# dariopagliaricci/Metal-PathTracer-arm64

Measured on AMD Instinct MI355X. Metric: Msamples/sec (whole node) at 1920×1080, depth 8; PFM RMSE vs Embree ref, higher is better.
Workload: dtype f32; 1 GPU; BASELINE configs[1]: Cornell box + one 70,688-triangle OBJ mesh, 1920x1080, depth 8, 256 spp, seed 1337; partition=8-row bands round-robin over 1 rank(s), RCCL gather of the HDR buffer

## Files before the change

### metal-pathtracer-arm64_amd/csrc/host/bvh_builder.cpp

```cpp
#include "bvh_builder.h"

#include <algorithm>
#include <atomic>
#include <cmath>
#include <chrono>
#include <cstdio>
#include <cstdlib>
#include <cstring>
#include <limits>
#include <memory>
#include <numeric>
#include <thread>
#include <stdexcept>

#if defined(__SSE2__)
#include <emmintrin.h>
#endif

#include "../kernels/bvh_layout.h"
#include "knobs.h"
#include "parallel.h"

namespace ptr {
namespace {
// ... 730 lines not shown
    for (int a = 0; a < 3; ++a) {
        const double extent = static_cast<double>(scene.hi[a]) - scene.lo[a];
        cell[a] = extent > 0.0 ? extent / 65531.0 : 1.0;
        out.gridCell[a] = static_cast<float>(cell[a]);
        out.gridOrigin[a] = static_cast<float>(scene.lo[a] - 2.0 * cell[a]);
    }
    out.qnodes.assign(static_cast<size_t>(out.nodeCount) * 8, 0u);
    auto quant = [&](float v, int axis, bool up) -> uint32_t {
        const double g = (static_cast<double>(v) - out.gridOrigin[axis]) / static_cast<double>(out.gridCell[axis]);
        const double q = up ? std::ceil(g) + 1.0 : std::floor(g) - 1.0;
        return static_cast<uint32_t>(std::min(std::max(q, 0.0), 65535.0));
    };
    auto quantiseRange = [&](uint32_t begin, uint32_t end) {
        for (uint32_t i = begin; i < end; ++i) {
            const float* n = out.nodes.data() + static_cast<size_t>(i) * 16;
            uint32_t* q = out.qnodes.data() + static_cast<size_t>(i) * 8;
            for (int c = 0; c < 2; ++c) {
                const float* lo = n + c * 8;
                const float* hi = n + c * 8 + 4;
                uint32_t ref;
                std::memcpy(&ref, n + (c == 0 ? 3 : 7), 4);
                uint32_t* w = q + c * 4;
                if (ref == ptrk::kRefEmpty) {
                    w[0] = w[1] = w[2] = 0u;
                } else {
                    w[0] = quant(lo[0], 0, false) | (quant(lo[1], 1, false) << 16);
                    w[1] = quant(lo[2], 2, false) | (quant(hi[0], 0, true) << 16);
                    w[2] = quant(hi[1], 1, true) | (quant(hi[2], 2, true) << 16);
                }
                w[3] = ref;
            }
        }
    };
    {
        const uint32_t workers = out.nodeCount >= (1u << 16) ? std::min(threads, 32u) : 1u;
        const uint32_t chunk = (out.nodeCount + workers - 1) / workers;
        runOnThreads(workers, [&](uint32_t t) {
            const uint32_t lo = std::min(out.nodeCount, chunk * t), hi = std::min(out.nodeCount, chunk * (t + 1));
            if (lo < hi) quantiseRange(lo, hi);
        });
    }
    double extentSum = 0.0;
    for (uint32_t i = 0; i < n; ++i) {
        const BuildPrim& p = prims[i];
        if (!oversize[i]) extentSum += std::max(std::max(p.hi[0] - p.lo[0], p.hi[1] - p.lo[1]), p.hi[2] - p.lo[2]);
    }
    out.meanPrimExtent = static_cast<float>(extentSum / std::max(inTree, 1u));
    lap("quantise");
}

namespace {

void emptyWidePlace(uint32_t* rec) {
    rec[0] = 0xFFFFFFFFu;
    rec[1] = 0x0000FFFFu;
    rec[2] = 0x00000000u;
    rec[3] = ptrk::kRefEmpty;
}

struct WideChoice {
    const uint32_t* rec[4];
    uint32_t count = 0;
};
inline bool internalRef(uint32_t ref, uint32_t nodeCount) { return ref != ptrk::kRefEmpty && !(ref & ptrk::kRefLeafBit) && ref < nodeCount; }
inline double quantArea(const uint32_t* rec, const float* cell) {
    const double x = (static_cast<double>(rec[1] >> 16) - (rec[0] & 0xFFFFu)) * cell[0];
    const double y = (static_cast<double>(rec[2] & 0xFFFFu) - (rec[0] >> 16)) * cell[1];
    const double z = (static_cast<double>(rec[2] >> 16) - (rec[1] & 0xFFFFu)) * cell[2];
    return x * y + y * z + z * x;
}
WideChoice chooseWideChildren(const uint32_t* q, uint32_t nodeCount, const float* cell, uint32_t n, bool byArea) {
    WideChoice c;
    auto childrenOf = [&](uint32_t node, const uint32_t** dst) {
        uint32_t got = 0;
        for (uint32_t side = 0; side < 2u; ++side) {
            const uint32_t* rec = q + static_cast<size_t>(node) * 8u + side * 4u;
            if (rec[3] != ptrk::kRefEmpty) dst[got++] = rec;
        }
        return got;
    };
    c.count = childrenOf(n, c.rec);
    if (!byArea) {
        WideChoice g;
        for (uint32_t k = 0; k < c.count; ++k) {
            if (internalRef(c.rec[k][3], nodeCount)) g.count += childrenOf(c.rec[k][3], g.rec + g.count);
            else g.rec[g.count++] = c.rec[k];
        }
        return g;
    }
    while (c.count < 4u) {
        int best = -1;
        double bestArea = -1.0;
        for (uint32_t k = 0; k < c.count; ++k) {
            if (!internalRef(c.rec[k][3], nodeCount)) continue;
            const double a = quantArea(c.rec[k], cell);
            if (a > bestArea) {
                bestArea = a;
                best = static_cast<int>(k);
            }
        }
        if (best < 0) break;
        const uint32_t* two[2];
        const uint32_t got = childrenOf(c.rec[best][3], two);
        if (got == 0u) break;
        c.rec[best] = two[0];
        if (got > 1u) c.rec[c.count++] = two[1];
    }
    return c;
}

}

uint32_t BuildWideNodes(const FlatBvh& bvh, WideCollapse how, std::unique_ptr<uint32_t[]>& wide, uint32_t* depthOut) {
    const uint32_t* q = bvh.qnodes.data();
    const uint32_t nodeCount = bvh.nodeCount;
    constexpr uint32_t kNotWide = 0xFFFFFFFFu;
    if (depthOut) *depthOut = 0u;
    if (nodeCount == 0 || bvh.qnodes.size() < static_cast<size_t>(nodeCount) * 8u) return 0;
    const bool byArea = how == WideCollapse::ByArea;
    std::unique_ptr<uint32_t[]> wideIndex(new uint32_t[nodeCount]);
    std::vector<uint8_t> depth(nodeCount, 0);
    depth[0] = 1u;
    uint32_t maxDepth = 1u;
    for (uint32_t n = 0; n < nodeCount; ++n) {
        if (depth[n] == 0u) continue;
        const WideChoice c = chooseWideChildren(q, nodeCount, bvh.gridCell, n, byArea);
        for (uint32_t k = 0; k < c.count; ++k) {
            const uint32_t ref = c.rec[k][3];
            if (internalRef(ref, nodeCount)) {
                depth[ref] = static_cast<uint8_t>(std::min<uint32_t>(depth[n] + 1u, 255u));
                maxDepth = std::max<uint32_t>(maxDepth, depth[ref]);
            }
        }
    }
    if (depthOut) *depthOut = maxDepth;
    uint32_t wideCount = 0;
    for (uint32_t n = 0; n < nodeCount; ++n) wideIndex[n] = depth[n] ? wideCount++ : kNotWide;
    wide.reset(new uint32_t[static_cast<size_t>(wideCount) * 16u]);
    const uint32_t workers = nodeCount >= (1u << 16) ? std::min(32u, std::max(1u, std::thread::hardware_concurrency())) : 1u;
    auto collapse = [&](uint32_t begin, uint32_t end) {
        for (uint32_t n = begin; n < end; ++n) {
            if (wideIndex[n] == kNotWide) continue;
            uint32_t* w = wide.get() + static_cast<size_t>(wideIndex[n]) * 16u;
            const WideChoice c = chooseWideChildren(q, nodeCount, bvh.gridCell, n, byArea);
            for (uint32_t k = 0; k < c.count; ++k) {
                uint32_t* dst = w + 4u * k;
                std::memcpy(dst, c.rec[k], 16);
                if (internalRef(dst[3], nodeCount)) dst[3] = wideIndex[dst[3]];
            }
            for (uint32_t k = c.count; k < 4u; ++k) emptyWidePlace(w + 4u * k);
        }
    };
    const uint32_t chunk = (nodeCount + workers - 1u) / workers;
    runOnThreads(workers, [&](uint32_t k) {
        const uint32_t b = std::min(nodeCount, chunk * k), e = std::min(nodeCount, chunk * (k + 1u));
        if (b < e) collapse(b, e);
    });
    return wideCount;
}

}
```

### metal-pathtracer-arm64_amd/csrc/host/cabi_host.cpp

```cpp
#include <algorithm>
#include <cmath>
#include <cstdio>
#include <cstring>
#include <exception>
#include <filesystem>
#include <memory>
#include <string>
#include <vector>

#include "env_importance_sampler.h"
#include "headless.h"
#include "image_decoders.h"
#include "image_writer.h"
#include "ptr_abi.h"
#include "ptr_debug.h"
#include "scene_geometry.h"
#include "bvh_layout.h"
#include "tangent_space.h"
#include "scene_manager.h"

struct PtrHostScene {
    ptr::SceneResources resources;
    ptr::RenderSettings settings;
    PtrSceneDesc desc{};
// ... 269 lines not shown
            for (int a = 0; a < 3; ++a) inv[a] = 1.0 / (d[a] != 0.0 ? d[a] : 1e-300);
            auto testLeaf = [&](uint32_t ref) {
                const uint32_t first = ref & ptrk::kRefOffsetMask, count = ((ref >> ptrk::kRefCountShift) & 0xFu) % ptrk::kMaxLeafPrims + 1u;
                for (uint32_t k = 0; k < count; ++k) {
                    ++prims;
                    if (ref & ptrk::kRefSphereBit) {
                        const float* sp = &geo.sphereData[static_cast<size_t>(first + k) * 4];
                        double c[3], dd = 0, b = 0, cc = 0;
                        for (int a = 0; a < 3; ++a) { c[a] = sp[a] - o[a]; dd += d[a] * d[a]; b += c[a] * d[a]; cc += c[a] * c[a]; }
                        const double disc = b * b - dd * (cc - static_cast<double>(sp[3]) * sp[3]);
                        if (disc < 0) continue;
                        const double sq = std::sqrt(disc);
                        double t = (b - sq) / dd;
                        if (t < tmin) t = (b + sq) / dd;
                        if (t >= tmin && t <= tfar) { tfar = t; hit = true; }
                    } else {
                        const float* t3 = &geo.triData[static_cast<size_t>(first + k) * 12];
                        const double v0[3] = {t3[0], t3[1], t3[2]}, e1[3] = {t3[4], t3[5], t3[6]}, e2[3] = {t3[8], t3[9], t3[10]};
                        const double ng[3] = {e2[1] * e1[2] - e2[2] * e1[1], e2[2] * e1[0] - e2[0] * e1[2], e2[0] * e1[1] - e2[1] * e1[0]};
                        const double c[3] = {v0[0] - o[0], v0[1] - o[1], v0[2] - o[2]};
                        const double rr[3] = {c[1] * d[2] - c[2] * d[1], c[2] * d[0] - c[0] * d[2], c[0] * d[1] - c[1] * d[0]};
                        const double den = ng[0] * d[0] + ng[1] * d[1] + ng[2] * d[2];
                        if (den == 0.0) continue;
                        const double sgn = den < 0 ? -1.0 : 1.0, ad = std::fabs(den);
                        const double U = (rr[0] * e2[0] + rr[1] * e2[1] + rr[2] * e2[2]) * sgn, V = (rr[0] * e1[0] + rr[1] * e1[1] + rr[2] * e1[2]) * sgn;
                        if (U < 0 || V < 0 || U + V > ad) continue;
                        const double T = (ng[0] * c[0] + ng[1] * c[1] + ng[2] * c[2]) * sgn;
                        if (!(ad * tmin < T && T <= ad * tfar)) continue;
                        tfar = T / ad;
                        hit = true;
                    }
                }
            };
            stack.clear();
            if (bvh.oversizeRef != ptrk::kRefEmpty) testLeaf(bvh.oversizeRef);
            if (bvh.rootRef != ptrk::kRefEmpty) stack.push_back(bvh.rootRef);
            while (!stack.empty()) {
                const uint32_t ref = stack.back();
                stack.pop_back();
                if (ref & ptrk::kRefLeafBit) {
                    testLeaf(ref);
                    continue;
                }
                ++steps;
                if (levels >= 5u) {
                    const uint32_t* w = wideNodes.get() + static_cast<size_t>(ref) * 16u;
                    double entry[4];
                    uint32_t order[4], on = 0, refs[4];
                    for (uint32_t k = 0; k < 4u; ++k) {
                        const uint32_t* rec = w + 4u * k;
                        refs[k] = rec[3];
                        if (rec[3] == ptrk::kRefEmpty) continue;
                        ++boxes;
                        const double lo[3] = {bvh.gridOrigin[0] + double(rec[0] & 0xFFFFu) * bvh.gridCell[0], bvh.gridOrigin[1] + double(rec[0] >> 16) * bvh.gridCell[1],
                                              bvh.gridOrigin[2] + double(rec[1] & 0xFFFFu) * bvh.gridCell[2]};
                        const double hi[3] = {bvh.gridOrigin[0] + double(rec[1] >> 16) * bvh.gridCell[0], bvh.gridOrigin[1] + double(rec[2] & 0xFFFFu) * bvh.gridCell[1],
                                              bvh.gridOrigin[2] + double(rec[2] >> 16) * bvh.gridCell[2]};
                        double t0 = tmin, t1 = tfar;
                        for (int a = 0; a < 3; ++a) {
                            const double ta = (lo[a] - o[a]) * inv[a], tb = (hi[a] - o[a]) * inv[a];
                            t0 = std::max(t0, std::min(ta, tb));
                            t1 = std::min(t1, std::max(ta, tb));
                        }
                        if (t0 <= t1) {
                            entry[k] = t0;
                            order[on++] = k;
                        }
                    }
                    std::sort(order, order + on, [&](uint32_t a, uint32_t b) { return entry[a] > entry[b]; });
                    for (uint32_t k = 0; k < on; ++k) stack.push_back(refs[order[k]]);
                    continue;
                }
                Child kids[8];
                uint32_t kn = 0;
                auto children = [&](uint32_t node, Child* dst) {
                    const float* nd = &bvh.nodes[static_cast<size_t>(node) * 16];
                    uint32_t c = 0;
                    for (int sl = 0; sl < 2; ++sl) {
                        const uint32_t cref = bits(nd[sl == 0 ? 3 : 7]);
                        if (cref != ptrk::kRefEmpty) dst[c++] = Child{nd + sl * 8, nd + sl * 8 + 4, cref};
                    }
                    return c;
                };
                kn = children(ref, kids);
                if (levels == 4u) {
                    auto area = [](const Child& c) {
                        const double x = double(c.hi[0]) - c.lo[0], y = double(c.hi[1]) - c.lo[1], z = double(c.hi[2]) - c.lo[2];
                        return x * y + y * z + z * x;
                    };
                    while (kn < 4u) {
                        int best = -1;
                        for (uint32_t k = 0; k < kn; ++k) {
                            if (!(kids[k].ref & ptrk::kRefLeafBit) && (best < 0 || area(kids[k]) > area(kids[best]))) best = static_cast<int>(k);
                        }
                        if (best < 0) break;
                        Child two[2];
                        const uint32_t got = children(kids[best].ref, two);
                        kids[best] = two[0];
                        if (got > 1u) kids[kn++] = two[1];
                    }
                }
                for (uint32_t l = 1; l < levels && levels != 4u; ++l) {
                    Child next[8];
                    uint32_t nn = 0;
                    for (uint32_t k = 0; k < kn; ++k) {
                        if (kids[k].ref & ptrk::kRefLeafBit) next[nn++] = kids[k];
                        else nn += children(kids[k].ref, next + nn);
                    }
                    std::memcpy(kids, next, sizeof(Child) * nn);
                    kn = nn;
// ... 31 lines not shown
```

### metal-pathtracer-arm64_amd/csrc/host/geometry_cache.cpp

```cpp
#include "geometry_cache.h"

#include <cstdio>
#include <cstring>
#include <vector>

namespace ptr {

namespace {

constexpr uint64_t kMagic = 0x3330454743525450ull;

struct Header {
    uint64_t magic, fingerprint;
    uint64_t nodes, qnodes, triOrder, sphereOrder, triData, triNormals, sphereData, sphereInfo, triUv, triTangent, rectTriLeaf, wideWords;
    float gridOrigin[3], gridCell[3], meanPrimExtent;
    uint32_t rootRef, oversizeRef, nodeCount, leafCount, maxDepth, maxLeafSize, triCount, sphereCount, useQuantized, wideCount, wideDepth, pad0;
    double sahCost, gatherSeconds, buildSeconds, flattenSeconds;
};

void fnv(uint64_t& h, const void* data, size_t bytes) {
    const unsigned char* p = static_cast<const unsigned char*>(data);
    for (size_t i = 0; i < bytes; ++i) {
        h ^= p[i];
        h *= 0x100000001b3ull;
    }
}

void fnvSampled(uint64_t& h, const void* data, size_t bytes) {
    const unsigned char* p = static_cast<const unsigned char*>(data);
    if (!p) return;
    const size_t piece = 4096;
    if (bytes <= 3 * piece) {
        fnv(h, p, bytes);
        return;
    }
    fnv(h, p, piece);
    fnv(h, p + (bytes / 2 / 16) * 16, piece);
    fnv(h, p + bytes - piece, piece);
}

template <typename T>
bool put(std::FILE* f, const T* data, uint64_t count) {
    return count == 0 || std::fwrite(data, sizeof(T), count, f) == count;
}

template <typename T>
bool get(std::FILE* f, std::vector<T>& v, uint64_t count) {
    v.resize(count);
    return count == 0 || std::fread(v.data(), sizeof(T), count, f) == count;
}

}

uint64_t SceneFingerprint(const PtrSceneDesc& desc) {
    uint64_t h = 0xcbf29ce484222325ull;
    fnv(h, &desc.meshCount, sizeof(desc.meshCount));
    for (uint32_t m = 0; m < desc.meshCount; ++m) {
        const PtrMeshDesc& mesh = desc.meshes[m];
        fnv(h, &mesh.vertexCount, sizeof(mesh.vertexCount));
        fnv(h, &mesh.indexCount, sizeof(mesh.indexCount));
        fnv(h, mesh.localToWorld, sizeof(mesh.localToWorld));
        fnv(h, &mesh.materialIndex, sizeof(mesh.materialIndex));
        fnvSampled(h, mesh.positions, static_cast<size_t>(mesh.vertexCount) * 12u);
// ... 129 lines not shown
```

### metal-pathtracer-arm64_amd/csrc/host/scene_geometry.cpp

```cpp
#include "scene_geometry.h"

#include <algorithm>
#include <atomic>
#include <chrono>
#include <cmath>
#include <cstdio>
#include <cstdlib>
#include <cstring>
#include <functional>
#include <thread>

#include "../kernels/bvh_layout.h"
#include "knobs.h"
#include "parallel.h"
#include "vecmath.h"

namespace ptr {
namespace {

struct M4 {
    float m[4][4];
};

M4 loadM4(const float* p) {
// ... 379 lines not shown
            } else {
                continue;
            }
            const float* lo = n + c * 8;
            const float* hi = n + c * 8 + 4;
            bool inside = true;
            for (int a = 0; a < 3; ++a) inside = inside && b.lo[a] >= lo[a] && b.hi[a] <= hi[a];
            if (!inside) out.boxViolations += 1;
            grow(subtree[ii], b.lo);
            grow(subtree[ii], b.hi);
            if (q) {
                const uint32_t* w = q + c * 4;
                const uint32_t qlo[3] = {w[0] & 0xFFFFu, w[0] >> 16, w[1] & 0xFFFFu};
                const uint32_t qhi[3] = {w[1] >> 16, w[2] & 0xFFFFu, w[2] >> 16};
                bool ok = (w[3] == ref);
                for (int a = 0; a < 3; ++a) {
                    const double dlo = static_cast<double>(bvh.gridOrigin[a]) + static_cast<double>(qlo[a]) * bvh.gridCell[a];
                    const double dhi = static_cast<double>(bvh.gridOrigin[a]) + static_cast<double>(qhi[a]) * bvh.gridCell[a];
                    ok = ok && dlo <= lo[a] && dhi >= hi[a];
                }
                if (!ok) out.quantViolations += 1;
            }
        }
    }
    if (bvh.oversizeRef != ptrk::kRefEmpty) {
        Box b{{inf, inf, inf}, {-inf, -inf, -inf}};
        if (!(bvh.oversizeRef & ptrk::kRefLeafBit) || (bvh.oversizeRef & ptrk::kRefSphereBit)) out.badRefs += 1;
        leafBounds(bvh.oversizeRef, b);
        out.oversize = ((bvh.oversizeRef >> ptrk::kRefCountShift) & 0xFu) + 1u;
    }
    for (uint8_t s : triSeen) out.unreferenced += (s == 0);
    for (uint8_t s : sphSeen) out.unreferenced += (s == 0);

    for (int pass = 0; pass < 2 && nodeCount > 0 && !bvh.qnodes.empty(); ++pass) {
        std::unique_ptr<uint32_t[]> wide;
        uint32_t wideDepth = 0;
        const uint32_t wideCount = BuildWideNodes(bvh, pass == 0 ? WideCollapse::ByArea : WideCollapse::ByLevel, wide, &wideDepth);
        if (pass == 0) {
            out.wideNodes = wideCount;
            out.wideDepth = wideDepth;
        }
        std::vector<uint8_t> triWide(g.triCount, 0), sphWide(g.sphereCount, 0), visited(wideCount, 0);
        std::vector<uint32_t> stack{0u};
        while (!stack.empty()) {
            const uint32_t n = stack.back();
            stack.pop_back();
            if (n >= wideCount || visited[n]++) {
                out.wideProblems += 1;
                continue;
            }
            for (uint32_t c = 0; c < 4u; ++c) {
                const uint32_t* rec = &wide[static_cast<size_t>(n) * 16u + c * 4u];
                const uint32_t ref = rec[3];
                const bool inverted = (rec[0] & 0xFFFFu) > (rec[1] >> 16) && (rec[0] >> 16) > (rec[2] & 0xFFFFu) && (rec[1] & 0xFFFFu) > (rec[2] >> 16);
                const bool ordered = (rec[0] & 0xFFFFu) <= (rec[1] >> 16) && (rec[0] >> 16) <= (rec[2] & 0xFFFFu) && (rec[1] & 0xFFFFu) <= (rec[2] >> 16);
                if ((ref == ptrk::kRefEmpty) ? !inverted : !ordered) out.wideProblems += 1;
                if (ref == ptrk::kRefEmpty) continue;
                if (!(ref & ptrk::kRefLeafBit)) {
                    stack.push_back(ref);
                    continue;
                }
                const uint32_t first = ref & ptrk::kRefOffsetMask, count = ((ref >> ptrk::kRefCountShift) & 0xFu) + 1u;
                std::vector<uint8_t>& seen = (ref & ptrk::kRefSphereBit) ? sphWide : triWide;
                for (uint32_t i = first; i < first + count; ++i) {
                    if (i >= seen.size() || seen[i]++) out.wideProblems += 1;
                }
            }
        }
        for (uint32_t n = 0; n < wideCount; ++n) out.wideProblems += (visited[n] == 0);
        const uint32_t outside = bvh.oversizeRef != ptrk::kRefEmpty ? ((bvh.oversizeRef >> ptrk::kRefCountShift) & 0xFu) + 1u : 0u;
        uint64_t missed = 0;
        for (uint8_t s : triWide) missed += (s == 0);
        for (uint8_t s : sphWide) missed += (s == 0);
        if (missed != outside) out.wideProblems += 1 + (missed > outside ? missed - outside : outside - missed);
    }
}

}
```

### metal-pathtracer-arm64_amd/csrc/kernels/traverse.h

```cpp
#pragma once

#include "device_types.h"
#include "vec.h"

namespace ptrk {

struct TraceCounters {
    uint32_t nodes;
    uint32_t prims;
    uint32_t waveNodeSteps = 0, wavePrimSteps = 0, leaves = 0;
};

typedef __attribute__((address_space(3))) uint32_t LdsWord;

struct LaneStack {
    LdsWord* lds;
    uint32_t* spill;
    uint32_t spillStride;
    uint32_t limit;
    uint32_t sp;
    __device__ __forceinline__ uint32_t* spillSlot(uint32_t level) const {
        const uint32_t column = blockIdx.x * kTraceBlock + threadIdx.x;
        return spill + static_cast<size_t>(level - kLdsStackLevels) * spillStride + column;
    }
    __device__ __forceinline__ void push(uint32_t v) {
        if (sp < kLdsStackLevels) {
            lds[sp * kTraceBlock] = v;
        } else if (sp < limit) {
            *spillSlot(sp) = v;
        } else {
            return;
        }
        ++sp;
    }
    __device__ __forceinline__ uint32_t pop() {
        --sp;
        return (sp < kLdsStackLevels) ? lds[sp * kTraceBlock] : *spillSlot(sp);
    }
};

typedef uint32_t u32x4 __attribute__((ext_vector_type(4)));

struct SceneMem {
    __amdgpu_buffer_rsrc_t nodes;
    __amdgpu_buffer_rsrc_t tris;
    __amdgpu_buffer_rsrc_t wide;
};

__device__ __forceinline__ SceneMem sceneMem(const SceneView& sc) {
    SceneMem m;
    const void* nodes = sc.useQuantized ? static_cast<const void*>(sc.qnodes) : static_cast<const void*>(sc.nodes);
    m.nodes = __builtin_amdgcn_make_buffer_rsrc(const_cast<void*>(nodes), 0, sc.nodeBytes, 0x00020000);
    m.tris = __builtin_amdgcn_make_buffer_rsrc(const_cast<float4*>(sc.tris), 0, sc.triBytes, 0x00020000);
    m.wide = __builtin_amdgcn_make_buffer_rsrc(const_cast<uint4*>(sc.wnodes), 0, sc.wideBytes, 0x00020000);
    return m;
}

__device__ __forceinline__ uint4 load16u(__amdgpu_buffer_rsrc_t r, uint32_t byteOffset) {
    const u32x4 v = __builtin_amdgcn_raw_buffer_load_b128(r, byteOffset, 0, 0);
    return make_uint4(v.x, v.y, v.z, v.w);
}
__device__ __forceinline__ float4 load16f(__amdgpu_buffer_rsrc_t r, uint32_t byteOffset) {
    const u32x4 v = __builtin_amdgcn_raw_buffer_load_b128(r, byteOffset, 0, 0);
    return make_float4(__uint_as_float(v.x), __uint_as_float(v.y), __uint_as_float(v.z), __uint_as_float(v.w));
}

struct TraceHit {
    float t;
    uint32_t prim;
};

typedef float v2f __attribute__((ext_vector_type(2)));

__device__ __forceinline__ bool slabTest(f3 lo, f3 hi, f3 oi, f3 inv, float tnear, float tfar, float& entry) {
    const v2f tx = __builtin_elementwise_fma((v2f){lo.x, hi.x}, (v2f){inv.x, inv.x}, (v2f){-oi.x, -oi.x});
    const v2f ty = __builtin_elementwise_fma((v2f){lo.y, hi.y}, (v2f){inv.y, inv.y}, (v2f){-oi.y, -oi.y});
    const v2f tz = __builtin_elementwise_fma((v2f){lo.z, hi.z}, (v2f){inv.z, inv.z}, (v2f){-oi.z, -oi.z});
    const float ax = tx.x, bx = tx.y, ay = ty.x, by = ty.y, az = tz.x, bz = tz.y;
    const float t0 = fmaxf(fmaxf(fminf(ax, bx), fminf(ay, by)), fmaxf(fminf(az, bz), tnear));
    const float t1 = fminf(fminf(fmaxf(ax, bx), fmaxf(ay, by)), fminf(fmaxf(az, bz), tfar));
    entry = t0;
    return t0 <= t1 * 1.0000004f;
}

__device__ __forceinline__ bool slabTestOrdered(f3 nearQ, f3 farQ, f3 oi, f3 inv, float tnear, float tfar, float& entry) {
    const v2f tx = __builtin_elementwise_fma((v2f){nearQ.x, farQ.x}, (v2f){inv.x, inv.x}, (v2f){-oi.x, -oi.x});
    const v2f ty = __builtin_elementwise_fma((v2f){nearQ.y, farQ.y}, (v2f){inv.y, inv.y}, (v2f){-oi.y, -oi.y});
    const v2f tz = __builtin_elementwise_fma((v2f){nearQ.z, farQ.z}, (v2f){inv.z, inv.z}, (v2f){-oi.z, -oi.z});
    const float t0 = fmaxf(fmaxf(tx.x, ty.x), fmaxf(tz.x, tnear));
    const float t1 = fminf(fminf(tx.y, ty.y), fminf(tz.y, tfar));
    entry = t0;
    return t0 <= t1 * 1.0000004f;
}

__device__ __forceinline__ bool triangleTest(f3 v0, f3 e1, f3 e2, f3 org, f3 dir, float tnear, float tfar,
                                             float& t, float& u, float& v) {
    const f3 Ng = cross(e2, e1);
    const f3 C = v0 - org;
    const f3 R = cross(C, dir);
    const float den = dot(Ng, dir);
    const float absDen = fabsf(den);
    const float sgn = signbit(den) ? -1.0f : 1.0f;
    const float U = dot(R, e2) * sgn;
    const float V = dot(R, e1) * sgn;
    if (!(den != 0.0f && U >= 0.0f && V >= 0.0f && (U + V) <= absDen)) return false;
    const float T = dot(Ng, C) * sgn;
    if (!(absDen * tnear < T && T <= absDen * tfar)) return false;
    const float rcpAbsDen = 1.0f / absDen;
    t = T * rcpAbsDen;
    u = U * rcpAbsDen;
    v = V * rcpAbsDen;
    return true;
}

__device__ __forceinline__ void triangleUv(f3 v0, f3 e1, f3 e2, f3 org, f3 dir, float& u, float& v) {
    const f3 Ng = cross(e2, e1);
    const f3 C = v0 - org;
    const f3 R = cross(C, dir);
    const float den = dot(Ng, dir);
    const float absDen = fabsf(den);
    const float sgn = signbit(den) ? -1.0f : 1.0f;
    const float U = dot(R, e2) * sgn;
    const float V = dot(R, e1) * sgn;
    const float rcpAbsDen = 1.0f / absDen;
    u = U * rcpAbsDen;
    v = V * rcpAbsDen;
}

__device__ __forceinline__ bool sphereTest(float4 s, f3 org, f3 dir, float tnear, float tfar, float& t) {
    const float rd2 = 1.0f / dot(dir, dir);
    const f3 c0 = mk3(s) - org;
    const float projC0 = dot(c0, dir) * rd2;
    const f3 perp = c0 - projC0 * dir;
    const float l2 = dot(perp, perp);
    const float r2 = s.w * s.w;
    if (!(l2 <= r2)) return false;
    const float td = sqrtf((r2 - l2) * rd2);
    const float tFront = projC0 - td;
    const float tBack = projC0 + td;
    const bool validFront = (tnear <= tFront) && (tFront <= tfar);
    const bool validBack = (tnear <= tBack) && (tBack <= tfar);
    if (!validFront && !validBack) return false;
    t = validFront ? tFront : tBack;
    return true;
}

struct Trav {
    f3 org, dir, inv;
    f3 oi;
    uint32_t selX, selY, selZ;
    float tnear;
    TraceHit hit;
    uint32_t cur;
    uint32_t leafPos;
    bool anyHit;
};

template <int NODES = -1>
__device__ __forceinline__ bool travBegin(const SceneView& sc, Trav& t, f3 org, f3 dir, float tnear, float tfar, bool anyHit,
                                          LaneStack& stack) {
    t.org = org;
    t.dir = dir;
    constexpr float kInvMax = 1.0e28f;
    t.inv = mk3(fminf(fmaxf(__builtin_amdgcn_rcpf(dir.x), -kInvMax), kInvMax), fminf(fmaxf(__builtin_amdgcn_rcpf(dir.y), -kInvMax), kInvMax),
                fminf(fmaxf(__builtin_amdgcn_rcpf(dir.z), -kInvMax), kInvMax));
    if (NODES >= 1 || (NODES < 0 && sc.useQuantized)) {
        const f3 cell = mk3(sc.gridCell[0], sc.gridCell[1], sc.gridCell[2]);
        const f3 invCell = mk3(sc.gridInvCell[0], sc.gridInvCell[1], sc.gridInvCell[2]);
        const f3 orgQ = (org - mk3(sc.gridOrigin[0], sc.gridOrigin[1], sc.gridOrigin[2])) * invCell;
        t.inv = t.inv * cell;
        t.oi = orgQ * t.inv;
    } else {
        t.oi = org * t.inv;
    }
    t.selX = t.inv.x < 0.0f ? 0x01000706u : 0x07060100u;
    t.selY = t.inv.y < 0.0f ? 0x03020504u : 0x05040302u;
    t.selZ = t.inv.z < 0.0f ? 0x01000706u : 0x07060100u;
    t.tnear = tnear;
    t.hit.t = tfar;
    t.hit.prim = kHitMiss;
    t.anyHit = anyHit;
    t.cur = sc.rootRef;
    t.leafPos = 0u;
    stack.sp = 0;
    if (sc.oversizeRef != kRefEmpty) {
        if (sc.rootRef != kRefEmpty) stack.push(sc.rootRef);
        t.cur = sc.oversizeRef;
        return true;
    }
    return sc.rootRef != kRefEmpty;
}

__device__ __forceinline__ bool travAtLeaf(const Trav& t) { return (t.cur & kRefLeafBit) != 0u; }
__device__ __forceinline__ bool travPop(Trav& t, LaneStack& stack) {
    if (stack.sp == 0) return false;
    t.cur = stack.pop();
    t.leafPos = 0u;
    return true;
}

__device__ __forceinline__ f3 gridLo(uint32_t w0, uint32_t w1) {
    return mk3(static_cast<float>(w0 & 0xFFFFu), static_cast<float>(w0 >> 16), static_cast<float>(w1 & 0xFFFFu));
}
__device__ __forceinline__ f3 gridHi(uint32_t w1, uint32_t w2) {
    return mk3(static_cast<float>(w1 >> 16), static_cast<float>(w2 & 0xFFFFu), static_cast<float>(w2 >> 16));
}

template <bool COUNT>
__device__ __forceinline__ bool travWideStep(const SceneMem& mem, Trav& t, LaneStack& stack, TraceCounters& cnt) {
    const uint32_t at = t.cur * 64u;
    const uint4 c0 = load16u(mem.wide, at), c1 = load16u(mem.wide, at + 16u), c2 = load16u(mem.wide, at + 32u), c3 = load16u(mem.wide, at + 48u);
    float k0, k1, k2, k3;
    auto boxTest = [&](const uint4& c, float& k) {
        const uint32_t wx = __builtin_amdgcn_perm(c.y, c.x, t.selX), wy = __builtin_amdgcn_perm(c.z, c.x, t.selY), wz = __builtin_amdgcn_perm(c.z, c.y, t.selZ);
        const f3 nearQ = mk3(static_cast<float>(wx & 0xFFFFu), static_cast<float>(wy & 0xFFFFu), static_cast<float>(wz & 0xFFFFu));
        const f3 farQ = mk3(static_cast<float>(wx >> 16), static_cast<float>(wy >> 16), static_cast<float>(wz >> 16));
        return slabTestOrdered(nearQ, farQ, t.oi, t.inv, t.tnear, t.hit.t, k);
    };
    const bool h0 = boxTest(c0, k0), h1 = boxTest(c1, k1), h2 = boxTest(c2, k2), h3 = boxTest(c3, k3);
    k0 = h0 ? k0 : INFINITY;
    k1 = h1 ? k1 : INFINITY;
    k2 = h2 ? k2 : INFINITY;
    k3 = h3 ? k3 : INFINITY;
    uint32_t r0 = c0.w, r1 = c1.w, r2 = c2.w, r3 = c3.w;
    if (COUNT) ++cnt.nodes;
    t.leafPos = 0u;
    auto exchange = [](float& ka, uint32_t& ra, float& kb, uint32_t& rb) {
        const bool swap = kb < ka;
        const float kLo = swap ? kb : ka, kHi = swap ? ka : kb;
        const uint32_t rLo = swap ? rb : ra, rHi = swap ? ra : rb;
        ka = kLo;
        kb = kHi;
        ra = rLo;
        rb = rHi;
    };
    exchange(k0, r0, k1, r1);
    exchange(k2, r2, k3, r3);
    exchange(k0, r0, k2, r2);
    exchange(k1, r1, k3, r3);
    exchange(k1, r1, k2, r2);
    if (k3 < INFINITY) stack.push(r3);
    if (k2 < INFINITY) stack.push(r2);
    if (k1 < INFINITY) stack.push(r1);
    if (k0 < INFINITY) {
        t.cur = r0;
        return true;
    }
    return travPop(t, stack);
}

template <bool COUNT, int NODES = -1>
__device__ __forceinline__ bool travNodeStep(const SceneView& sc, const SceneMem& mem, Trav& t, LaneStack& stack, TraceCounters& cnt) {
    if (NODES == 2) return travWideStep<COUNT>(mem, t, stack, cnt);
    uint32_t ref0, ref1;
    float e0, e1;
    bool h0, h1;
    if (NODES == 1 || (NODES < 0 && sc.useQuantized)) {
        const uint4 q0 = load16u(mem.nodes, t.cur * 32u), q1 = load16u(mem.nodes, t.cur * 32u + 16u);
        ref0 = q0.w;
        ref1 = q1.w;
        h0 = slabTest(gridLo(q0.x, q0.y), gridHi(q0.y, q0.z), t.oi, t.inv, t.tnear, t.hit.t, e0);
        h1 = slabTest(gridLo(q1.x, q1.y), gridHi(q1.y, q1.z), t.oi, t.inv, t.tnear, t.hit.t, e1);
    } else {
        const uint32_t at = t.cur * 64u;
        const float4 n0 = load16f(mem.nodes, at), n1 = load16f(mem.nodes, at + 16u), n2 = load16f(mem.nodes, at + 32u),
                     n3 = load16f(mem.nodes, at + 48u);
        ref0 = __float_as_uint(n0.w);
        ref1 = __float_as_uint(n1.w);
        h0 = slabTest(mk3(n0), mk3(n1), t.oi, t.inv, t.tnear, t.hit.t, e0);
        h1 = slabTest(mk3(n2), mk3(n3), t.oi, t.inv, t.tnear, t.hit.t, e1);
// ... 106 lines not shown
```

Before: 2532 Msamples/s.

## Repack wide BVH boxes per axis and decode planes via biased-float perm

Wide BVH child records now store each axis's lo/hi pair in one 32-bit word instead of interleaving axes across words. The traversal kernel builds each box plane as a float directly with a byte perm against the 2^23 bias exponent, so it skips the integer mask/shift and int-to-float conversions. The ray origin term is folded into a precomputed biased offset. A host-side checker is added to compare culling against the old formulation. The geometry cache magic is bumped, and the bias trick risks precision loss for far-away rays.

After: 2561 Msamples/s (median of 6 runs). 1.01x the previous value.

```diff
diff --git a/metal-pathtracer-arm64_amd/csrc/host/bvh_builder.cpp b/metal-pathtracer-arm64_amd/csrc/host/bvh_builder.cpp
--- a/metal-pathtracer-arm64_amd/csrc/host/bvh_builder.cpp
+++ b/metal-pathtracer-arm64_amd/csrc/host/bvh_builder.cpp
@@ -806,10 +806,15 @@
 namespace {
 
 void emptyWidePlace(uint32_t* rec) {
-    rec[0] = 0xFFFFFFFFu;
-    rec[1] = 0x0000FFFFu;
-    rec[2] = 0x00000000u;
+    rec[0] = rec[1] = rec[2] = 0x0000FFFFu;
     rec[3] = ptrk::kRefEmpty;
+}
+
+void wideRecord(const uint32_t* bin, uint32_t* rec) {
+    rec[0] = (bin[0] & 0xFFFFu) | (bin[1] & 0xFFFF0000u);
+    rec[1] = (bin[0] >> 16) | (bin[2] << 16);
+    rec[2] = (bin[1] & 0xFFFFu) | (bin[2] & 0xFFFF0000u);
+    rec[3] = bin[3];
 }
 
 struct WideChoice {
@@ -899,7 +904,7 @@
             const WideChoice c = chooseWideChildren(q, nodeCount, bvh.gridCell, n, byArea);
             for (uint32_t k = 0; k < c.count; ++k) {
                 uint32_t* dst = w + 4u * k;
-                std::memcpy(dst, c.rec[k], 16);
+                wideRecord(c.rec[k], dst);
                 if (internalRef(dst[3], nodeCount)) dst[3] = wideIndex[dst[3]];
             }
             for (uint32_t k = c.count; k < 4u; ++k) emptyWidePlace(w + 4u * k);
diff --git a/metal-pathtracer-arm64_amd/csrc/host/cabi_host.cpp b/metal-pathtracer-arm64_amd/csrc/host/cabi_host.cpp
--- a/metal-pathtracer-arm64_amd/csrc/host/cabi_host.cpp
+++ b/metal-pathtracer-arm64_amd/csrc/host/cabi_host.cpp
@@ -345,10 +345,11 @@
                         refs[k] = rec[3];
                         if (rec[3] == ptrk::kRefEmpty) continue;
                         ++boxes;
-                        const double lo[3] = {bvh.gridOrigin[0] + double(rec[0] & 0xFFFFu) * bvh.gridCell[0], bvh.gridOrigin[1] + double(rec[0] >> 16) * bvh.gridCell[1],
-                                              bvh.gridOrigin[2] + double(rec[1] & 0xFFFFu) * bvh.gridCell[2]};
-                        const double hi[3] = {bvh.gridOrigin[0] + double(rec[1] >> 16) * bvh.gridCell[0], bvh.gridOrigin[1] + double(rec[2] & 0xFFFFu) * bvh.gridCell[1],
-                                              bvh.gridOrigin[2] + double(rec[2] >> 16) * bvh.gridCell[2]};
+                        double lo[3], hi[3];
+                        for (int a = 0; a < 3; ++a) {
+                            lo[a] = bvh.gridOrigin[a] + double(rec[a] & 0xFFFFu) * bvh.gridCell[a];
+                            hi[a] = bvh.gridOrigin[a] + double(rec[a] >> 16) * bvh.gridCell[a];
+                        }
                         double t0 = tmin, t1 = tfar;
                         for (int a = 0; a < 3; ++a) {
                             const double ta = (lo[a] - o[a]) * inv[a], tb = (hi[a] - o[a]) * inv[a];
diff --git a/metal-pathtracer-arm64_amd/csrc/host/geometry_cache.cpp b/metal-pathtracer-arm64_amd/csrc/host/geometry_cache.cpp
--- a/metal-pathtracer-arm64_amd/csrc/host/geometry_cache.cpp
+++ b/metal-pathtracer-arm64_amd/csrc/host/geometry_cache.cpp
@@ -8,7 +8,7 @@
 
 namespace {
 
-constexpr uint64_t kMagic = 0x3330454743525450ull;
+constexpr uint64_t kMagic = 0x3430454743525450ull;
 
 struct Header {
     uint64_t magic, fingerprint;
diff --git a/metal-pathtracer-arm64_amd/csrc/host/scene_geometry.cpp b/metal-pathtracer-arm64_amd/csrc/host/scene_geometry.cpp
--- a/metal-pathtracer-arm64_amd/csrc/host/scene_geometry.cpp
+++ b/metal-pathtracer-arm64_amd/csrc/host/scene_geometry.cpp
@@ -455,8 +455,8 @@
             for (uint32_t c = 0; c < 4u; ++c) {
                 const uint32_t* rec = &wide[static_cast<size_t>(n) * 16u + c * 4u];
                 const uint32_t ref = rec[3];
-                const bool inverted = (rec[0] & 0xFFFFu) > (rec[1] >> 16) && (rec[0] >> 16) > (rec[2] & 0xFFFFu) && (rec[1] & 0xFFFFu) > (rec[2] >> 16);
-                const bool ordered = (rec[0] & 0xFFFFu) <= (rec[1] >> 16) && (rec[0] >> 16) <= (rec[2] & 0xFFFFu) && (rec[1] & 0xFFFFu) <= (rec[2] >> 16);
+                const bool inverted = (rec[0] & 0xFFFFu) > (rec[0] >> 16) && (rec[1] & 0xFFFFu) > (rec[1] >> 16) && (rec[2] & 0xFFFFu) > (rec[2] >> 16);
+                const bool ordered = (rec[0] & 0xFFFFu) <= (rec[0] >> 16) && (rec[1] & 0xFFFFu) <= (rec[1] >> 16) && (rec[2] & 0xFFFFu) <= (rec[2] >> 16);
                 if ((ref == ptrk::kRefEmpty) ? !inverted : !ordered) out.wideProblems += 1;
                 if (ref == ptrk::kRefEmpty) continue;
                 if (!(ref & ptrk::kRefLeafBit)) {
diff --git a/metal-pathtracer-arm64_amd/csrc/host/wide_check.cpp b/metal-pathtracer-arm64_amd/csrc/host/wide_check.cpp
--- /dev/null
+++ b/metal-pathtracer-arm64_amd/csrc/host/wide_check.cpp
@@ -0,0 +1,244 @@
+#include <algorithm>
+#include <atomic>
+#include <cmath>
+#include <cstdint>
+#include <cstdio>
+#include <cstring>
+#include <string>
+#include <thread>
+#include <vector>
+
+#include "bvh_builder.h"
+#include "bvh_layout.h"
+#include "parallel.h"
+#include "ptr_abi.h"
+#include "scene_geometry.h"
+#include "wide_box.h"
+
+namespace {
+
+struct V3 {
+    float x, y, z;
+};
+inline V3 sub(V3 a, V3 b) { return V3{a.x - b.x, a.y - b.y, a.z - b.z}; }
+inline V3 mul(V3 a, V3 b) { return V3{a.x * b.x, a.y * b.y, a.z * b.z}; }
+inline float dot(V3 a, V3 b) { return (a.x * b.x + a.y * b.y) + a.z * b.z; }
+inline V3 cross(V3 a, V3 b) { return V3{a.y * b.z - a.z * b.y, a.z * b.x - a.x * b.z, a.x * b.y - a.y * b.x}; }
+
+bool triangleTest(V3 v0, V3 e1, V3 e2, V3 org, V3 dir, float tnear, float tfar, float& t) {
+    const V3 Ng = cross(e2, e1);
+    const V3 C = sub(v0, org);
+    const V3 R = cross(C, dir);
+    const float den = dot(Ng, dir);
+    const float absDen = std::fabs(den);
+    const float sgn = std::signbit(den) ? -1.0f : 1.0f;
+    const float U = dot(R, e2) * sgn;
+    const float V = dot(R, e1) * sgn;
+    if (!(den != 0.0f && U >= 0.0f && V >= 0.0f && (U + V) <= absDen)) return false;
+    const float T = dot(Ng, C) * sgn;
+    if (!(absDen * tnear < T && T <= absDen * tfar)) return false;
+    t = T * (1.0f / absDen);
+    return true;
+}
+
+struct SplitMix {
+    uint64_t s;
+    uint64_t next() {
+        uint64_t z = (s += 0x9E3779B97F4A7C15ull);
+        z = (z ^ (z >> 30)) * 0xBF58476D1CE4E5B9ull;
+        z = (z ^ (z >> 27)) * 0x94D049BB133111EBull;
+        return z ^ (z >> 31);
+    }
+    float uniform() { return static_cast<float>(next() >> 40) * (1.0f / 16777216.0f); }
+};
+
+}
+
+extern "C" {
+
+int ptr_debug_wide_check(const PtrSceneDesc* scene, const float* rays, uint64_t n, uint64_t extra, uint64_t out[6], char* err, size_t errCap) {
+    auto fail = [&](const std::string& msg) {
+        if (err && errCap) std::snprintf(err, errCap, "%s", msg.c_str());
+        return 1;
+    };
+    try {
+        if (!scene || (!rays && n) || !out) return fail("ptr_debug_wide_check: bad argument");
+        ptr::SceneGeometry geo;
+        std::string error;
+        if (!ptr::BuildSceneGeometry(*scene, 0, geo, error)) return fail(error);
+        const ptr::FlatBvh& bvh = geo.bvh;
+        std::unique_ptr<uint32_t[]> wide;
+        const uint32_t wideCount = bvh.nodeCount > 0 ? ptr::BuildWideNodes(bvh, ptr::WideCollapse::ByArea, wide) : 0u;
+        if (wideCount == 0) return fail("ptr_debug_wide_check: scene without four-wide nodes");
+        constexpr uint32_t kNone = 0xFFFFFFFFu;
+        std::vector<uint32_t> nodeOwner(wideCount, kNone), triOwner(geo.triCount, kNone);
+        for (uint32_t w = 0; w < wideCount; ++w) {
+            for (uint32_t k = 0; k < 4u; ++k) {
+                const uint32_t ref = wide[w * 16u + k * 4u + 3u];
+                if (ref == ptrk::kRefEmpty) continue;
+                if (!(ref & ptrk::kRefLeafBit)) {
+                    nodeOwner[ref] = (w << 2) | k;
+                } else if (!(ref & ptrk::kRefSphereBit)) {
+                    const uint32_t first = ref & ptrk::kRefOffsetMask, count = ((ref >> ptrk::kRefCountShift) & 0xFu) + 1u;
+                    for (uint32_t i = first; i < first + count && i < geo.triCount; ++i) triOwner[i] = (w << 2) | k;
+                }
+            }
+        }
+        auto tri = [&](uint32_t i, int c) {
+            const float* p = &geo.triData[static_cast<size_t>(i) * 12 + c * 4];
+            return V3{p[0], p[1], p[2]};
+        };
+
+        std::vector<float> all(rays, rays + n * 8);
+        std::vector<uint32_t> inTree;
+        for (uint32_t i = 0; i < geo.triCount; ++i) {
+            if (triOwner[i] != kNone) inTree.push_back(i);
+        }
+        SplitMix rng{12345u};
+        const float cellMax = std::max(std::max(bvh.gridCell[0], bvh.gridCell[1]), bvh.gridCell[2]);
+        for (uint64_t r = 0; r < extra * 5u && !inTree.empty(); ++r) {
+            const int kind = static_cast<int>(r % 5u);
+            const uint32_t ti = inTree[rng.next() % inTree.size()];
+            const V3 v0 = tri(ti, 0), e1 = tri(ti, 1), e2 = tri(ti, 2);
+            float b1 = rng.uniform(), b2 = rng.uniform();
+            if (b1 + b2 > 1.0f) { b1 = 1.0f - b1; b2 = 1.0f - b2; }
+            V3 p{v0.x - b1 * e1.x + b2 * e2.x, v0.y - b1 * e1.y + b2 * e2.y, v0.z - b1 * e1.z + b2 * e2.z};
+            float d[3] = {rng.uniform() * 2.0f - 1.0f, rng.uniform() * 2.0f - 1.0f, rng.uniform() * 2.0f - 1.0f};
+            const int axis = static_cast<int>(rng.next() % 3u);
+            float dist = (0.001f + rng.uniform()) * cellMax * 65536.0f * 0.5f;
+            if (kind == 0) {
+                d[axis] = (rng.next() & 1u) ? 0.0f : -0.0f;
+                if (rng.next() & 1u) d[(axis + 1) % 3] = (rng.next() & 1u) ? 0.0f : -0.0f;
+            } else if (kind == 1) {
+                const int c = static_cast<int>(rng.next() % 3u);
+                p = c == 0 ? v0 : c == 1 ? sub(v0, e1) : V3{v0.x + e2.x, v0.y + e2.y, v0.z + e2.z};
+                d[axis] = (rng.next() & 1u) ? 0.0f : -0.0f;
+            } else if (kind == 3) {
+                dist = cellMax * std::ldexp(1.0f, 20 + static_cast<int>(rng.next() % 12u));
+            }
+            float len = std::sqrt(d[0] * d[0] + d[1] * d[1] + d[2] * d[2]);
+            if (!(len > 0.0f)) { d[axis] = 1.0f; len = 1.0f; }
+            for (float& c : d) c /= len;
+            float o[3] = {p.x - dist * d[0], p.y - dist * d[1], p.z - dist * d[2]};
+            if (kind == 4) {
+                for (int a = 0; a < 3; ++a) o[a] = bvh.gridOrigin[a] + (rng.uniform() * 1.2f - 0.1f) * 65536.0f * bvh.gridCell[a];
+                if (rng.next() & 1u) {
+                    const float to[3] = {p.x - o[0], p.y - o[1], p.z - o[2]};
+                    const float l = std::sqrt(to[0] * to[0] + to[1] * to[1] + to[2] * to[2]);
+                    if (l > 0.0f) for (int a = 0; a < 3; ++a) d[a] = to[a] / l;
+                }
+            }
+            if (kind == 2) {
+                for (int a = 0; a < 3; ++a) {
+                    const float k = std::round((o[a] - bvh.gridOrigin[a]) / bvh.gridCell[a]);
+                    o[a] = bvh.gridOrigin[a] + k * bvh.gridCell[a];
+                }
+            }
+            const float ray[8] = {o[0], o[1], o[2], 1e-4f, d[0], d[1], d[2], INFINITY};
+            all.insert(all.end(), ray, ray + 8);
+        }
+        const uint64_t total = all.size() / 8;
+
+        std::atomic<uint64_t> farRays{0}, pairs{0}, misses{0}, farMisses{0}, both{0};
+        const uint32_t threads = std::max(1u, std::min(16u, std::thread::hardware_concurrency()));
+        ptr::runOnThreads(threads, [&](uint32_t th) {
+            uint64_t myFar = 0, myPairs = 0, myMisses = 0, myFarMisses = 0, myBoth = 0;
+            std::vector<uint32_t> stack;
+            for (uint64_t r = th; r < total; r += threads) {
+                const float* q = &all[r * 8];
+                const V3 org{q[0], q[1], q[2]}, dir{q[4], q[5], q[6]};
+                const float tnear = q[3], tfar = q[7];
+                const float dd[3] = {dir.x, dir.y, dir.z};
+                float inv[3];
+                for (int a = 0; a < 3; ++a) {
+                    float rc = 1.0f / dd[a];
+                    const int wiggle = static_cast<int>((r * 3u + static_cast<uint64_t>(a)) % 3u) - 1;
+                    if (std::isfinite(rc) && wiggle != 0) rc = std::nextafter(rc, wiggle > 0 ? INFINITY : -INFINITY);
+                    inv[a] = std::fmin(std::fmax(rc, -1.0e28f), 1.0e28f) * bvh.gridCell[a];
+                }
+                const V3 invCell{1.0f / bvh.gridCell[0], 1.0f / bvh.gridCell[1], 1.0f / bvh.gridCell[2]};
+                const V3 orgQ = mul(sub(org, V3{bvh.gridOrigin[0], bvh.gridOrigin[1], bvh.gridOrigin[2]}), invCell);
+                const float oq[3] = {orgQ.x, orgQ.y, orgQ.z};
+                float bias[3];
+                uint32_t selN[3];
+                for (int a = 0; a < 3; ++a) {
+                    bias[a] = ptrk::wideBias(oq[a], inv[a]);
+                    selN[a] = ptrk::wideSelNear(inv[a]);
+                }
+                myFar += (std::fabs(oq[0]) > 65536.0f || std::fabs(oq[1]) > 65536.0f || std::fabs(oq[2]) > 65536.0f) ? 1u : 0u;
+                const bool veryFar = std::fabs(oq[0]) >= 16777216.0f || std::fabs(oq[1]) >= 16777216.0f || std::fabs(oq[2]) >= 16777216.0f;
+                const double od[3] = {org.x, org.y, org.z};
+                stack.assign(1, 0u);
+                while (!stack.empty()) {
+                    const uint32_t w = stack.back();
+                    stack.pop_back();
+                    for (uint32_t k = 0; k < 4u; ++k) {
+                        const uint32_t* rec = &wide[w * 16u + k * 4u];
+                        if (rec[3] == ptrk::kRefEmpty) continue;
+                        double t0 = tnear, t1 = INFINITY;
+                        for (int a = 0; a < 3 && t0 <= t1; ++a) {
+                            const double lo = bvh.gridOrigin[a] + (double(rec[a] & 0xFFFFu) - 8.0) * bvh.gridCell[a];
+                            const double hi = bvh.gridOrigin[a] + (double(rec[a] >> 16) + 8.0) * bvh.gridCell[a];
+                            if (dd[a] == 0.0f) {
+                                if (od[a] < lo || od[a] > hi) t0 = INFINITY;
+                                continue;
+                            }
+                            const double ta = (lo - od[a]) / dd[a], tb = (hi - od[a]) / dd[a];
+                            t0 = std::max(t0, std::min(ta, tb));
+                            t1 = std::min(t1, std::max(ta, tb));
+                        }
+                        if (!(t0 <= t1)) continue;
+                        if (!(rec[3] & ptrk::kRefLeafBit)) {
+                            stack.push_back(rec[3]);
+                            continue;
+                        }
+                        if (rec[3] & ptrk::kRefSphereBit) continue;
+                        const uint32_t first = rec[3] & ptrk::kRefOffsetMask, count = ((rec[3] >> ptrk::kRefCountShift) & 0xFu) + 1u;
+                        for (uint32_t i = first; i < first + count; ++i) {
+                            float th;
+                            if (!triangleTest(tri(i, 0), tri(i, 1), tri(i, 2), org, dir, tnear, tfar, th)) continue;
+                            ++myPairs;
+                            bool culled = false, culledBefore = false;
+                            for (uint32_t at = triOwner[i]; at != kNone; at = nodeOwner[at >> 2]) {
+                                const uint32_t* box = &wide[(at >> 2) * 16u + (at & 3u) * 4u];
+                                float entry;
+                                if (!ptrk::wideBoxTest(box, inv, bias, selN, tnear, th, entry)) culled = true;
+                                float n3[3], f3[3];
+                                for (int a = 0; a < 3; ++a) {
+                                    const float lo = static_cast<float>(box[a] & 0xFFFFu), hi = static_cast<float>(box[a] >> 16);
+                                    const float oi = oq[a] * inv[a];
+                                    n3[a] = std::fmaf(inv[a] < 0.0f ? hi : lo, inv[a], -oi);
+                                    f3[a] = std::fmaf(inv[a] < 0.0f ? lo : hi, inv[a], -oi);
+                                }
+                                const float t0 = std::fmax(std::fmax(n3[0], n3[1]), std::fmax(n3[2], tnear));
+                                const float t1 = std::fmin(std::fmin(f3[0], f3[1]), std::fmin(f3[2], th));
+                                if (!(t0 <= t1 * 1.0000004f)) culledBefore = true;
+                                if ((at >> 2) == 0u) break;
+                            }
+                            myBoth += (culled && culledBefore) ? 1u : 0u;
+                            (veryFar ? myFarMisses : myMisses) += (culled && !culledBefore) ? 1u : 0u;
+                        }
+                    }
+                }
+            }
+            farRays += myFar;
+            pairs += myPairs;
+            misses += myMisses;
+            both += myBoth;
+            farMisses += myFarMisses;
+        });
+        out[0] = total;
+        out[1] = farRays.load();
+        out[2] = pairs.load();
+        out[3] = misses.load();
+        out[4] = both.load();
+        out[5] = farMisses.load();
+        return 0;
+    } catch (const std::exception& e) {
+        return fail(e.what());
+    } catch (...) {
+        return fail("ptr_debug_wide_check: unknown error");
+    }
+}
+
+}
diff --git a/metal-pathtracer-arm64_amd/csrc/kernels/traverse.h b/metal-pathtracer-arm64_amd/csrc/kernels/traverse.h
--- a/metal-pathtracer-arm64_amd/csrc/kernels/traverse.h
+++ b/metal-pathtracer-arm64_amd/csrc/kernels/traverse.h
@@ -2,6 +2,7 @@
 
 #include "device_types.h"
 #include "vec.h"
+#include "wide_box.h"
 
 namespace ptrk {
 
@@ -79,16 +80,6 @@
     const float ax = tx.x, bx = tx.y, ay = ty.x, by = ty.y, az = tz.x, bz = tz.y;
     const float t0 = fmaxf(fmaxf(fminf(ax, bx), fminf(ay, by)), fmaxf(fminf(az, bz), tnear));
     const float t1 = fminf(fminf(fmaxf(ax, bx), fmaxf(ay, by)), fminf(fmaxf(az, bz), tfar));
-    entry = t0;
-    return t0 <= t1 * 1.0000004f;
-}
-
-__device__ __forceinline__ bool slabTestOrdered(f3 nearQ, f3 farQ, f3 oi, f3 inv, float tnear, float tfar, float& entry) {
-    const v2f tx = __builtin_elementwise_fma((v2f){nearQ.x, farQ.x}, (v2f){inv.x, inv.x}, (v2f){-oi.x, -oi.x});
-    const v2f ty = __builtin_elementwise_fma((v2f){nearQ.y, farQ.y}, (v2f){inv.y, inv.y}, (v2f){-oi.y, -oi.y});
-    const v2f tz = __builtin_elementwise_fma((v2f){nearQ.z, farQ.z}, (v2f){inv.z, inv.z}, (v2f){-oi.z, -oi.z});
-    const float t0 = fmaxf(fmaxf(tx.x, ty.x), fmaxf(tz.x, tnear));
-    const float t1 = fminf(fminf(tx.y, ty.y), fminf(tz.y, tfar));
     entry = t0;
     return t0 <= t1 * 1.0000004f;
 }
@@ -169,13 +160,17 @@
         const f3 invCell = mk3(sc.gridInvCell[0], sc.gridInvCell[1], sc.gridInvCell[2]);
         const f3 orgQ = (org - mk3(sc.gridOrigin[0], sc.gridOrigin[1], sc.gridOrigin[2])) * invCell;
         t.inv = t.inv * cell;
-        t.oi = orgQ * t.inv;
+        if (NODES == 2) {
+            t.oi = mk3(wideBias(orgQ.x, t.inv.x), wideBias(orgQ.y, t.inv.y), wideBias(orgQ.z, t.inv.z));
+            t.selX = wideSelNear(t.inv.x);
+            t.selY = wideSelNear(t.inv.y);
+            t.selZ = wideSelNear(t.inv.z);
+        } else {
+            t.oi = orgQ * t.inv;
+        }
     } else {
         t.oi = org * t.inv;
     }
-    t.selX = t.inv.x < 0.0f ? 0x01000706u : 0x07060100u;
-    t.selY = t.inv.y < 0.0f ? 0x03020504u : 0x05040302u;
-    t.selZ = t.inv.z < 0.0f ? 0x01000706u : 0x07060100u;
     t.tnear = tnear;
     t.hit.t = tfar;
     t.hit.prim = kHitMiss;
@@ -211,11 +206,20 @@
     const uint32_t at = t.cur * 64u;
     const uint4 c0 = load16u(mem.wide, at), c1 = load16u(mem.wide, at + 16u), c2 = load16u(mem.wide, at + 32u), c3 = load16u(mem.wide, at + 48u);
     float k0, k1, k2, k3;
+    auto other = [](uint32_t sel) {
+        uint32_t r;
+        asm volatile("v_xor_b32 %0, 0x202, %1" : "=v"(r) : "v"(sel));
+        return r;
+    };
+    const uint32_t farX = other(t.selX), farY = other(t.selY), farZ = other(t.selZ);
     auto boxTest = [&](const uint4& c, float& k) {
-        const uint32_t wx = __builtin_amdgcn_perm(c.y, c.x, t.selX), wy = __builtin_amdgcn_perm(c.z, c.x, t.selY), wz = __builtin_amdgcn_perm(c.z, c.y, t.selZ);
-        const f3 nearQ = mk3(static_cast<float>(wx & 0xFFFFu), static_cast<float>(wy & 0xFFFFu), static_cast<float>(wz & 0xFFFFu));
-        const f3 farQ = mk3(static_cast<float>(wx >> 16), static_cast<float>(wy >> 16), static_cast<float>(wz >> 16));
-        return slabTestOrdered(nearQ, farQ, t.oi, t.inv, t.tnear, t.hit.t, k);
+        const v2f tx = __builtin_elementwise_fma((v2f){widePlane(c.x, t.selX), widePlane(c.x, farX)}, (v2f){t.inv.x, t.inv.x}, (v2f){-t.oi.x, -t.oi.x});
+        const v2f ty = __builtin_elementwise_fma((v2f){widePlane(c.y, t.selY), widePlane(c.y, farY)}, (v2f){t.inv.y, t.inv.y}, (v2f){-t.oi.y, -t.oi.y});
+        const v2f tz = __builtin_elementwise_fma((v2f){widePlane(c.z, t.selZ), widePlane(c.z, farZ)}, (v2f){t.inv.z, t.inv.z}, (v2f){-t.oi.z, -t.oi.z});
+        const float t0 = fmaxf(fmaxf(tx.x, ty.x), fmaxf(tz.x, t.tnear));
+        const float t1 = fminf(fminf(tx.y, ty.y), fminf(tz.y, t.hit.t));
+        k = t0;
+        return t0 <= t1 * 1.0000004f;
     };
     const bool h0 = boxTest(c0, k0), h1 = boxTest(c1, k1), h2 = boxTest(c2, k2), h3 = boxTest(c3, k3);
     k0 = h0 ? k0 : INFINITY;
diff --git a/metal-pathtracer-arm64_amd/csrc/kernels/wide_box.h b/metal-pathtracer-arm64_amd/csrc/kernels/wide_box.h
--- /dev/null
+++ b/metal-pathtracer-arm64_amd/csrc/kernels/wide_box.h
@@ -0,0 +1,81 @@
+#pragma once
+
+#include <cmath>
+#include <cstdint>
+#include <cstring>
+
+#if defined(__HIPCC__)
+#define PTR_WIDE_FN __host__ __device__ __forceinline__
+#else
+#define PTR_WIDE_FN inline
+#endif
+
+namespace ptrk {
+
+constexpr uint32_t kWideBiasBits = 0x4B000000u;
+constexpr float kWideBias = 8388608.0f;
+constexpr uint32_t kWideSelLow = 0x070C0100u;
+constexpr uint32_t kWideSelHigh = 0x070C0302u;
+constexpr uint32_t kWideSelOther = 0x0202u;
+
+PTR_WIDE_FN uint32_t wideFloatBits(float f) {
+#if defined(__HIP_DEVICE_COMPILE__)
+    return __float_as_uint(f);
+#else
+    uint32_t u;
+    std::memcpy(&u, &f, 4);
+    return u;
+#endif
+}
+PTR_WIDE_FN float wideBitsFloat(uint32_t u) {
+#if defined(__HIP_DEVICE_COMPILE__)
+    return __uint_as_float(u);
+#else
+    float f;
+    std::memcpy(&f, &u, 4);
+    return f;
+#endif
+}
+
+PTR_WIDE_FN uint32_t widePerm(uint32_t hi, uint32_t lo, uint32_t sel) {
+#if defined(__HIP_DEVICE_COMPILE__)
+    return __builtin_amdgcn_perm(hi, lo, sel);
+#else
+    const uint64_t v = (static_cast<uint64_t>(hi) << 32) | lo;
+    uint32_t r = 0;
+    for (int i = 0; i < 4; ++i) {
+        const uint32_t s = (sel >> (8 * i)) & 0xFFu;
+        const uint32_t byte = s < 8u ? static_cast<uint32_t>(v >> (8 * s)) & 0xFFu : 0u;
+        r |= byte << (8 * i);
+    }
+    return r;
+#endif
+}
+
+PTR_WIDE_FN float wideFma(float a, float b, float c) {
+#if defined(__HIP_DEVICE_COMPILE__)
+    return __builtin_fmaf(a, b, c);
+#else
+    return std::fmaf(a, b, c);
+#endif
+}
+
+PTR_WIDE_FN float wideBias(float orgQ, float inv) { return wideFma(orgQ, inv, kWideBias * inv); }
+PTR_WIDE_FN uint32_t wideSelNear(float inv) { return inv < 0.0f ? kWideSelHigh : kWideSelLow; }
+
+PTR_WIDE_FN float widePlane(uint32_t word, uint32_t sel) { return wideBitsFloat(widePerm(kWideBiasBits, word, sel)); }
+
+PTR_WIDE_FN bool wideBoxTest(const uint32_t rec[3], const float inv[3], const float bias[3], const uint32_t selN[3], float tnear, float tfar,
+                             float& entry) {
+    float n[3], f[3];
+    for (int a = 0; a < 3; ++a) {
+        n[a] = wideFma(widePlane(rec[a], selN[a]), inv[a], -bias[a]);
+        f[a] = wideFma(widePlane(rec[a], selN[a] ^ kWideSelOther), inv[a], -bias[a]);
+    }
+    const float t0 = std::fmax(std::fmax(n[0], n[1]), std::fmax(n[2], tnear));
+    const float t1 = std::fmin(std::fmin(f[0], f[1]), std::fmin(f[2], tfar));
+    entry = t0;
+    return t0 <= t1 * 1.0000004f;
+}
+
+}
```
